# stm233/image-compression-for-machine

Measured on AMD Instinct MI355X. Metric: images/sec (256x256) cnn-hyperprior (WACNN) training step, higher is better.
Workload: dtype f32; 1 GPU; cnn (WACNN N=192 M=320) train step, lambda=0.0067 MSE, batch 16/GPU synthetic 256x256, Adam lr 1e-4 + aux Adam, clip 1.0; global_batch=16, parallelism=dp1

## Files before the change

image-compression-for-machine_amd/csrc/conv_1x1.hip:

```cpp
#include <cstdlib>
#include "conv_common.h"

namespace icm {

template <int TCO, int TPX>
__global__ __launch_bounds__(256, 2) void conv1x1_kernel(const ConvDesc d) {
  constexpr int DB = 4;
  const int lane = threadIdx.x & 63;
  const int wave = __builtin_amdgcn_readfirstlane((int)(threadIdx.x >> 6));
  const ConvPtrs P = d.g[blockIdx.y];
  int bid = xcd_block_id();
  const int cb = bid % d.ncb, ptile = bid / d.ncb;
  const int h = lane >> 5, l31 = lane & 31;
  const int HW = d.pg.H * d.pg.W;
  const int NP = d.pg.N * HW;
  const int p_base = (ptile * 4 + wave) * (32 * TPX);
  if (p_base >= NP) return;
  unsigned voff[TPX];
  int pn[TPX], phw[TPX];
  bool pv[TPX];
#pragma unroll
  for (int tp = 0; tp < TPX; ++tp) {
    const int p = p_base + tp * 32 + l31;
    pv[tp] = p < NP;
    const int pc = min(p, NP - 1);
    pn[tp] = pc / HW;
    phw[tp] = pc - pn[tp] * HW;
    voff[tp] = (unsigned)(pn[tp] * (int)d.pg.bs + phw[tp] + h * HW) * 4u;
  }
  f32x16 acc[TCO][TPX];
#pragma unroll
  for (int a = 0; a < TCO; ++a)
#pragma unroll
    for (int b = 0; b < TPX; ++b)
#pragma unroll
      for (int r = 0; r < 16; ++r) acc[a][b][r] = 0.0f;

  const char* xb = reinterpret_cast<const char*>(P.x);
  const char* wbase = reinterpret_cast<const char*>(P.wp);
  const long long cstride = (long long)HW * 4;
  const int cot0 = cb * TCO;
  unsigned wl[TCO];
#pragma unroll
  for (int a = 0; a < TCO; ++a) wl[a] = (unsigned)(min(cot0 + a, d.ncot - 1) * 64 + lane) * 16u;
  const long long qstride = (long long)d.ncot * 64 * 16;
  const int nq = d.nchunks8;
  const int act = d.pg.act;

  float bq[DB][4][TPX];
  f32x4 aq[2][TCO];
  auto loadB = [&](float (&dst)[4][TPX], int q) {
    const char* sb = xb + (long long)min(q, nq - 1) * 8 * cstride;
#pragma unroll
    for (int j = 0; j < 4; ++j)
#pragma unroll
      for (int tp = 0; tp < TPX; ++tp) dst[j][tp] = *reinterpret_cast<const float*>(sb + 2 * j * cstride + voff[tp]);
  };
#pragma unroll
  for (int a = 0; a < TCO; ++a) {
    aq[0][a] = *reinterpret_cast<const f32x4*>(wbase + wl[a]);
    aq[1][a] = *reinterpret_cast<const f32x4*>(wbase + (long long)min(1, nq - 1) * qstride + wl[a]);
  }
#pragma unroll
  for (int u = 0; u < DB; ++u) loadB(bq[u], u);

  for (int q0 = 0; q0 < nq; q0 += DB) {
#pragma unroll
    for (int u = 0; u < DB; ++u) {
      const int q = q0 + u;
      if (q >= nq) break;
      float bv[4][TPX];
#pragma unroll
      for (int j = 0; j < 4; ++j)
#pragma unroll
        for (int tp = 0; tp < TPX; ++tp) bv[j][tp] = bq[u][j][tp];
      if (act == ICM_ACT_GELU) {
#pragma unroll
        for (int j = 0; j < 4; ++j)
#pragma unroll
          for (int tp = 0; tp < TPX; ++tp) bv[j][tp] = gelu_f(bv[j][tp]);
      } else if (act == ICM_ACT_SQUARE) {
#pragma unroll
        for (int j = 0; j < 4; ++j)
#pragma unroll
          for (int tp = 0; tp < TPX; ++tp) bv[j][tp] *= bv[j][tp];
      }
      loadB(bq[u], q + DB);
      const char* sp = wbase + (long long)min(q + 2, nq - 1) * qstride;
#pragma unroll
      for (int a = 0; a < TCO; ++a) {
#pragma unroll
        for (int tp = 0; tp < TPX; ++tp)
#pragma unroll
          for (int j = 0; j < 4; ++j)
            acc[a][tp] = __builtin_amdgcn_mfma_f32_32x32x2f32(aq[u & 1][a][j], bv[j][tp], acc[a][tp], 0, 0, 0);
        aq[u & 1][a] = *reinterpret_cast<const f32x4*>(sp + wl[a]);
        __builtin_amdgcn_sched_barrier(0);
      }
    }
  }

  int zero[TPX];
#pragma unroll
  for (int tp = 0; tp < TPX; ++tp) zero[tp] = 0;
  epilogue_dispatch<TCO, TPX, !(TCO == 3 && TPX == 2)>(d, P, acc, cot0, h, pn, zero, phw, pv);
}

struct Cfg1x1 {
  int tco, tpx;
  void (*fn)(const ConvDesc);
  float eff;
};
static const Cfg1x1 kCfgs1x1[] = {
    {6, 1, conv1x1_kernel<6, 1>, 1.0f},  {5, 1, conv1x1_kernel<5, 1>, 1.0f}, {4, 1, conv1x1_kernel<4, 1>, 0.97f},
    {3, 2, conv1x1_kernel<3, 2>, 1.0f},  {2, 2, conv1x1_kernel<2, 2>, 0.7f}, {1, 2, conv1x1_kernel<1, 2>, 0.6f},
    {3, 1, conv1x1_kernel<3, 1>, 0.95f}, {2, 1, conv1x1_kernel<2, 1>, 0.6f},
};

int plan_conv1x1(const icm_conv_args& a, int ngroups, int g_force_1x1, ConvPlan& p) {
  if (g_force_1x1 == 0) return -1;
  if (a.KH != 1 || a.KW != 1 || a.stride != 1 || a.pad != 0 || a.pixel_shuffle || (a.Cin % 8) != 0) return -1;
  if (a.OH != a.H || a.OW != a.W) return -1;
  const int ncot = cdiv(a.Cout, 32);
  const long long NP = (long long)a.N * a.H * a.W;
  int best = -1, best_pad = 1 << 30;
  const int ncfg = (int)(sizeof(kCfgs1x1) / sizeof(kCfgs1x1[0]));
  for (int i = 0; i < ncfg; ++i) best_pad = std::min(best_pad, cdiv(ncot, kCfgs1x1[i].tco) * kCfgs1x1[i].tco);
  float best_score = -1.0f;
  for (int i = 0; i < ncfg; ++i) {
    const Cfg1x1& k = kCfgs1x1[i];
    if (cdiv(ncot, k.tco) * k.tco != best_pad) continue;
    const long long waves = ((NP + 32 * k.tpx - 1) / (32 * k.tpx)) * cdiv(ncot, k.tco) * ngroups;
    const float score = (float)std::min<long long>(waves, 2048) * k.eff;
    if (score > best_score) {
      best_score = score;
      best = i;
    }
  }
  {
    static const int force = env_int("ICM_1X1_CFG", -1);
    if (force >= 0 && force < ncfg) best = force;
  }
  const Cfg1x1& c = kCfgs1x1[best];
  const int ncb = cdiv(ncot, c.tco);
  const long long strips = (NP + 32 * c.tpx - 1) / (32 * c.tpx);
  static const long long kMinWaves = env_ll("ICM_1X1_MIN_WAVES", 1024);
  static const int kShortK = env_int("ICM_1X1_SHORT_K", 384);
  const long long need = a.Cin <= kShortK ? kMinWaves / 2 : kMinWaves;
  if (g_force_1x1 < 0 && strips * ncb * ngroups < need) return -1;
  const long long nblk = ((strips + 3) / 4) * ncb;
  if (nblk <= 0 || nblk > 0x7fffffffLL) return ICM_ERR_ARG;
  p = ConvPlan{};
  p.family = kFam1x1; p.row = best; p.g.ckm = 1; p.ncb = ncb; p.nblk = nblk; p.block = 256;
  return ICM_OK;
}

int launch_conv1x1(ConvDesc& d, const icm_conv_args& a, const ConvPlan& p, int ngroups, hipStream_t stream) {
  d.pg.H = a.H; d.pg.W = a.W; d.pg.N = a.N; d.pg.C = a.Cin; d.pg.act = a.pro_act; d.pg.bs = a.x_bs;
  d.OHf = a.H; d.OWf = a.W; d.OHv = a.H; d.OWv = a.W;
  d.out_sy = d.out_sx = 1;
  d.ntaps = 1;
  d.tiles_x = d.tiles_y = d.tiles_n = 1;
  d.nchunks8 = a.Cin / 8; d.ckm = p.g.ckm;
  hipLaunchKernelGGL(kCfgs1x1[p.row].fn, dim3((unsigned)p.nblk, ngroups, 1), dim3(p.block), 0, stream, d);
  ICM_CHECK_LAUNCH();
  return ICM_OK;
}

}
```

image-compression-for-machine_amd/csrc/conv_common.h:

```cpp
#pragma once
#include <type_traits>
#include "icm_common.h"

namespace icm {

#define ICM_MAX_TAPS 32
#define ICM_MAX_GROUPS 12

struct ConvPtrs {
  const float* x;
  const float* wp;
  const float* bias;
  float* y;
  const float* res;
  const float* aux;
  const float* aux2;
  float* y2;
};

struct ConvDesc {
  ConvPtrs g[ICM_MAX_GROUPS];
  long long y_bs, res_bs, aux_bs, aux2_bs, y2_bs;
  PatchGeom pg;
  int Cout, OHf, OWf;
  int OHv, OWv;
  int out_sy, out_oy, out_sx, out_ox;
  int iy0, ix0;
  int ntaps;
  int lgTW, lgTH, lgTI;
  int tiles_x, tiles_y, tiles_n;
  int ncot, nchunks8, ckm, ncb;
  int epi, accum, ps2;
  int tapoff[ICM_MAX_TAPS];
};

inline void fill_conv_ptrs(ConvPtrs (&g)[ICM_MAX_GROUPS], const icm_conv_args* arr, int ngroups, long long wp_off) {
  for (int gi = 0; gi < ICM_MAX_GROUPS; ++gi) {
    const icm_conv_args& s = arr[gi < ngroups ? gi : 0];
    g[gi] = ConvPtrs{s.x, s.wp + wp_off, s.bias, s.y, s.res, s.aux, s.aux2, s.y2};
  }
}
inline void fill_conv_desc(ConvDesc& d, const icm_conv_args* arr, int ngroups, long long wp_off) {
  const icm_conv_args& a = arr[0];
  fill_conv_ptrs(d.g, arr, ngroups, wp_off);
  d.y_bs = a.y_bs; d.res_bs = a.res_bs; d.aux_bs = a.aux_bs; d.aux2_bs = a.aux2_bs; d.y2_bs = a.y2_bs;
  d.Cout = a.Cout; d.ncot = (a.Cout + 31) / 32;
  d.epi = a.epi; d.accum = a.accum;
}

enum ConvFamily { kFamStaged = 0, kFamKs8 = 1, kFam1x1 = 2, kFamWino44 = 3, kFamWino8 = 4 };
struct Geometry {
  int lgTW, lgTH, lgTI, PH, PW, PWh, PWrow, PP, CS, tiles_x, tiles_y, tiles_n, ckm;
  size_t lds_bytes;
};
struct ConvPlan {
  int family;
  int row;
  Geometry g;
  int ncb;
  long long nblk;
  int block, vec4, dma;
};
struct WinoGeom {
  int lgTX, lgTY, lgTI, tiles_x, tiles_y, tiles_n, nchunks8, nsteps;
};
struct WinoPlan {
  WinoGeom g;
  int tco, w8, px_fast, ncb;
  long long nblk;
  size_t lds_bytes;
};

constexpr bool epi_reads_res(int e) { return e == ICM_EPI_RES || e == ICM_EPI_RES_GELU || e == ICM_EPI_RES_MUL_DGELU; }
constexpr bool epi_reads_aux(int e) {
  return e == ICM_EPI_GDN || e == ICM_EPI_IGDN || e == ICM_EPI_MUL_DGELU || e == ICM_EPI_AXPY2 || e == ICM_EPI_LRP ||
         e == ICM_EPI_RES_MUL_DGELU;
}
constexpr bool epi_reads_aux2(int e) { return e == ICM_EPI_AXPY2; }
constexpr bool epi_writes_side(int e) { return e == ICM_EPI_GDN || e == ICM_EPI_IGDN || e == ICM_EPI_LRP; }
constexpr bool epi_may_gelu(int e) { return e == ICM_EPI_NONE || e == ICM_EPI_RES || e == ICM_EPI_RES_GELU; }

template <int EPI>
__device__ __forceinline__ float epi_apply(float v, float rv, float av, float& side) {
  if constexpr (EPI == ICM_EPI_RES) v += rv;
  if constexpr (EPI == ICM_EPI_RES_GELU) v += gelu_f(rv);
  if constexpr (EPI == ICM_EPI_GDN || EPI == ICM_EPI_IGDN) {
    side = v;
    v = av * (EPI == ICM_EPI_GDN ? rsqrtf(v) : sqrtf(v));
  }
  if constexpr (EPI == ICM_EPI_MUL_DGELU) v *= dgelu_f(av);
  if constexpr (EPI == ICM_EPI_RES_MUL_DGELU) v = (v + rv) * dgelu_f(av);
  if constexpr (EPI == ICM_EPI_AXPY2) v = rv + 2.0f * av * v;
  if constexpr (EPI == ICM_EPI_LRP) {
    side = tanhf(v);
    v = av + 0.5f * side;
  }
  return v;
}
template <class Off>
__device__ __forceinline__ void epi_materialise(float& v, const float* y, float* y2, Off off, bool ok) {
  const float gv = gelu_f(v);
  if (y2 == y) v = gv;
  else if (ok) y2[off] = gv;
}

template <int... Kinds>
struct EpiKinds {
  static constexpr bool has(int epi) { return ((epi == Kinds) || ...); }
  template <class F>
  static __device__ __forceinline__ void dispatch(int epi, F&& f) {
    static_assert(((Kinds == ICM_EPI_NONE) || ...), "ICM_EPI_NONE is the fallback of every kernel");
    const bool hit = ((Kinds != ICM_EPI_NONE && epi == Kinds ? (f(std::integral_constant<int, Kinds>{}), true) : false) || ...);
    if (!hit) f(std::integral_constant<int, ICM_EPI_NONE>{});
  }
};
using EpiAll = EpiKinds<ICM_EPI_NONE, ICM_EPI_RES, ICM_EPI_RES_GELU, ICM_EPI_GDN, ICM_EPI_IGDN, ICM_EPI_MUL_DGELU,
                        ICM_EPI_AXPY2, ICM_EPI_LRP, ICM_EPI_RES_MUL_DGELU>;
using EpiKs8 = EpiKinds<ICM_EPI_NONE, ICM_EPI_RES, ICM_EPI_RES_GELU, ICM_EPI_MUL_DGELU, ICM_EPI_LRP, ICM_EPI_RES_MUL_DGELU>;
using EpiWino = EpiKinds<ICM_EPI_NONE, ICM_EPI_RES, ICM_EPI_RES_GELU, ICM_EPI_MUL_DGELU, ICM_EPI_RES_MUL_DGELU, ICM_EPI_LRP>;

template <int EPI, int half>
__device__ __forceinline__ void store_half_e(const ConvDesc& d, const ConvPtrs& P, const f32x16 acc, int cot, int h,
                                             int n, int oy, int ox, bool pvalid) {
  const int plane = d.OHf * d.OWf;
  constexpr bool kRes = epi_reads_res(EPI), kAux = epi_reads_aux(EPI), kAux2 = epi_reads_aux2(EPI);
  float* yb = P.y + n * d.y_bs;
  const float* resb = kRes ? P.res + n * d.res_bs : nullptr;
  const float* auxb = kAux ? P.aux + n * d.aux_bs : nullptr;
  const float* aux2b = kAux2 ? P.aux2 + n * d.aux2_bs : nullptr;
  float* y2b = P.y2 ? P.y2 + n * d.y2_bs : nullptr;
  const bool has_bias = P.bias != nullptr;
  {
    int off[8];
    bool ok[8];
    float bv[8], rv[8], av[8];
#pragma unroll
    for (int q = 0; q < 8; ++q) {
      const int r = half * 8 + q;
      const int co = cot * 32 + (r & 3) + 8 * (r >> 2) + 4 * h;
      ok[q] = pvalid && co < d.Cout;
      off[q] = d.ps2 ? (co >> 2) * plane + (oy * 2 + ((co >> 1) & 1)) * d.OWf + ox * 2 + (co & 1)
                     : co * plane + oy * d.OWf + ox;
      bv[q] = (has_bias && ok[q]) ? P.bias[co] : 0.0f;
      if constexpr (kRes) rv[q] = ok[q] ? resb[off[q]] : 0.0f;
      if constexpr (kAux) av[q] = ok[q] ? auxb[off[q]] : 0.0f;
      if constexpr (kAux2) rv[q] = ok[q] ? aux2b[off[q]] : 0.0f;
    }
    float v[8];
#pragma unroll
    for (int q = 0; q < 8; ++q) {
      float side;
      v[q] = epi_apply<EPI>(acc[half * 8 + q] + bv[q], (kRes || kAux2) ? rv[q] : 0.0f, kAux ? av[q] : 0.0f, side);
      if constexpr (epi_writes_side(EPI))
        if (y2b && ok[q]) y2b[off[q]] = side;
    }
    if (d.accum) {
      float old[8];
#pragma unroll
      for (int q = 0; q < 8; ++q) old[q] = ok[q] ? yb[off[q]] : 0.0f;
#pragma unroll
      for (int q = 0; q < 8; ++q) v[q] += old[q];
    }
    if constexpr (epi_may_gelu(EPI)) {
      if (y2b) {
#pragma unroll
        for (int q = 0; q < 8; ++q) epi_materialise(v[q], yb, y2b, off[q], ok[q]);
      }
    }
#pragma unroll
    for (int q = 0; q < 8; ++q)
      if (ok[q]) yb[off[q]] = v[q];
  }
}
template <int EPI>
__device__ __forceinline__ void store_tile_e(const ConvDesc& d, const ConvPtrs& P, const f32x16 acc, int cot, int h,
                                             int n, int oy, int ox, bool pvalid) {
  store_half_e<EPI, 0>(d, P, acc, cot, h, n, oy, ox, pvalid);
  store_half_e<EPI, 1>(d, P, acc, cot, h, n, oy, ox, pvalid);
}

struct EpiRegs {
  int n;
  int off[8];
  bool ok[8];
  float bv[8], rv[8], av[8], old[8];
};

template <int EPI>
__device__ __forceinline__ void epi_load(const ConvDesc& d, const ConvPtrs& P, int cot, int half, int h, int n, int oy,
                                         int ox, bool pvalid, EpiRegs& R) {
  const int plane = d.OHf * d.OWf;
  constexpr bool kRes = epi_reads_res(EPI), kAux = epi_reads_aux(EPI), kAux2 = epi_reads_aux2(EPI);
  const float* yb = P.y + n * d.y_bs;
  const float* resb = kRes ? P.res + n * d.res_bs : nullptr;
  const float* auxb = kAux ? P.aux + n * d.aux_bs : nullptr;
  const float* aux2b = kAux2 ? P.aux2 + n * d.aux2_bs : nullptr;
  const bool has_bias = P.bias != nullptr;
  const bool tile_ok = pvalid && cot < d.ncot;
  R.n = n;
#pragma unroll
  for (int q = 0; q < 8; ++q) {
    const int r = half * 8 + q;
    const int co = cot * 32 + (r & 3) + 8 * (r >> 2) + 4 * h;
    R.ok[q] = tile_ok && co < d.Cout;
    R.off[q] = d.ps2 ? (co >> 2) * plane + (oy * 2 + ((co >> 1) & 1)) * d.OWf + ox * 2 + (co & 1)
                     : co * plane + oy * d.OWf + ox;
    R.bv[q] = (has_bias && R.ok[q]) ? P.bias[co] : 0.0f;
    if constexpr (kRes) R.rv[q] = R.ok[q] ? resb[R.off[q]] : 0.0f;
    if constexpr (kAux) R.av[q] = R.ok[q] ? auxb[R.off[q]] : 0.0f;
    if constexpr (kAux2) R.rv[q] = R.ok[q] ? aux2b[R.off[q]] : 0.0f;
  }
  if (d.accum) {
#pragma unroll
    for (int q = 0; q < 8; ++q) R.old[q] = R.ok[q] ? yb[R.off[q]] : 0.0f;
  }
}

template <int EPI>
__device__ __forceinline__ void epi_finish(const ConvDesc& d, const ConvPtrs& P, const float (&a8)[8], const EpiRegs& R) {
  float* yb = P.y + R.n * d.y_bs;
  float* y2b = P.y2 ? P.y2 + R.n * d.y2_bs : nullptr;
  constexpr bool kRv = epi_reads_res(EPI) || epi_reads_aux2(EPI), kAux = epi_reads_aux(EPI);
  float v[8];
#pragma unroll
  for (int q = 0; q < 8; ++q) {
    float side;
    v[q] = epi_apply<EPI>(a8[q] + R.bv[q], kRv ? R.rv[q] : 0.0f, kAux ? R.av[q] : 0.0f, side);
    if constexpr (epi_writes_side(EPI))
      if (y2b && R.ok[q]) y2b[R.off[q]] = side;
  }
  if (d.accum) {
#pragma unroll
    for (int q = 0; q < 8; ++q) v[q] += R.old[q];
  }
  if constexpr (epi_may_gelu(EPI)) {
    if (y2b) {
#pragma unroll
      for (int q = 0; q < 8; ++q) epi_materialise(v[q], yb, y2b, R.off[q], R.ok[q]);
    }
  }
#pragma unroll
  for (int q = 0; q < 8; ++q)
    if (R.ok[q]) yb[R.off[q]] = v[q];
}

template <int EPI, int TCO, int TPX, bool PIPE>
__device__ __forceinline__ void epilogue_tiles(const ConvDesc& d, const ConvPtrs& P, const f32x16 (&acc)[TCO][TPX], int cot0,
                                               int h, const int (&pn)[TPX], const int (&poy)[TPX], const int (&pox)[TPX],
                                               const bool (&pv)[TPX]) {
  if constexpr (!PIPE) {
#pragma unroll
    for (int tp = 0; tp < TPX; ++tp)
#pragma unroll
      for (int a = 0; a < TCO; ++a) {
        if (cot0 + a < d.ncot) store_tile_e<EPI>(d, P, acc[a][tp], cot0 + a, h, pn[tp], poy[tp], pox[tp], pv[tp]);
        __builtin_amdgcn_sched_barrier(0);
      }
    return;
  }
  constexpr int S = TPX * TCO * 2;
  EpiRegs R[2];
  epi_load<EPI>(d, P, cot0, 0, h, pn[0], poy[0], pox[0], pv[0], R[0]);
#pragma unroll
  for (int i = 0; i < S; ++i) {
    const int half = i & 1, a = (i >> 1) % TCO, tp = (i >> 1) / TCO;
    if (i + 1 < S) {
      const int i2 = i + 1;
      const int half2 = i2 & 1, a2 = (i2 >> 1) % TCO, tp2 = (i2 >> 1) / TCO;
      epi_load<EPI>(d, P, cot0 + a2, half2, h, pn[tp2], poy[tp2], pox[tp2], pv[tp2], R[i2 & 1]);
    }
    __builtin_amdgcn_sched_barrier(0);
    float a8[8];
#pragma unroll
    for (int q = 0; q < 8; ++q) a8[q] = acc[a][tp][half * 8 + q];
    epi_finish<EPI>(d, P, a8, R[i & 1]);
    __builtin_amdgcn_sched_barrier(0);
  }
}

template <int TCO, int TPX, bool PIPE2 = false>
__device__ __forceinline__ void epilogue_dispatch(const ConvDesc& d, const ConvPtrs& P, const f32x16 (&acc)[TCO][TPX],
                                                  int cot0, int h, const int (&pn)[TPX], const int (&poy)[TPX],
                                                  const int (&pox)[TPX], const bool (&pv)[TPX]) {
  EpiAll::dispatch(d.epi, [&](auto kind) {
    constexpr int EPI = decltype(kind)::value;
    epilogue_tiles<EPI, TCO, TPX, EPI == ICM_EPI_AXPY2 && PIPE2>(d, P, acc, cot0, h, pn, poy, pox, pv);
  });
}

int launch_conv_ks8(const ConvDesc& d, int tco, long long nblk, int ngroups, size_t lds_bytes, hipStream_t stream);

bool wino_supported(const icm_conv_args& a);
int plan_conv_wino(const icm_conv_args& a, int ngroups, WinoPlan& p);
int run_conv_wino(const icm_conv_args* arr, int ngroups, hipStream_t stream);
long long wino_transform_floats(const icm_conv_args& a);
int run_wino_transform(const icm_conv_args* arr, int ngroups, hipStream_t stream);

int plan_conv1x1(const icm_conv_args& a, int ngroups, int force_mode, ConvPlan& p);
int launch_conv1x1(ConvDesc& d, const icm_conv_args& a, const ConvPlan& p, int ngroups, hipStream_t stream);

}
```

image-compression-for-machine_amd/csrc/conv_ks8.hip:

```cpp
#include <cstdlib>
#include "conv_common.h"

namespace icm {

template <int EPI>
__device__ __forceinline__ void ks8_store(const ConvDesc& d, const ConvPtrs& P, const f32x16 v, int cot, int hf, int h, int n,
                                          int oy, int ox, bool pvalid) {
  if (hf == 0) store_half_e<EPI, 0>(d, P, v, cot, h, n, oy, ox, pvalid);
  else store_half_e<EPI, 1>(d, P, v, cot, h, n, oy, ox, pvalid);
}

template <int TCO, int TPX>
__global__ __launch_bounds__(512, 2) void conv_ks8_kernel(const ConvDesc d) {
  extern __shared__ __attribute__((aligned(16))) float smem[];
  static_assert(TCO * TPX == 4, "four output tiles per workgroup: one half tile per wave in the epilogue");
  const int tid = threadIdx.x, lane = tid & 63;
  const int wave = __builtin_amdgcn_readfirstlane(tid >> 6);
  const ConvPtrs P = d.g[blockIdx.y];
  const PatchGeom& pg = d.pg;
  int bid = xcd_block_id();
  const int cb = bid % d.ncb;
  int pt = bid / d.ncb;
  const int tx_i = pt % d.tiles_x;
  pt /= d.tiles_x;
  const int ty_i = pt % d.tiles_y;
  const int tn_i = pt / d.tiles_y;
  const int ox0 = tx_i << d.lgTW, oy0 = ty_i << d.lgTH, n0 = tn_i << d.lgTI;
  const int iyb = oy0 + d.iy0, ixb = ox0 + d.ix0;
  const int bufsz = d.ckm * 8 * pg.CS;
  const int nchunks = (d.nchunks8 + d.ckm - 1) / d.ckm;
  const long long HWb = (long long)pg.H * pg.W * 4;
  const float* zero = icm_zero_page + lane;
  const int nj = (pg.TIPH * pg.PW + 63) >> 6;

  PlaneMap pm;
  plane_map_init(pm, pg, n0, iyb, ixb, lane);
  const char* xb = reinterpret_cast<const char*>(P.x);
  auto stage = [&](int chunk) {
    const int c0 = chunk * d.ckm * 8;
    const int nch = min(d.ckm, d.nchunks8 - chunk * d.ckm) * 8;
    float* dst = smem + (chunk & 1) * bufsz;
    for (int cl = wave; cl < nch; cl += 8) {
      const int c = c0 + cl;
      const char* base = xb + (long long)c * HWb;
      float* slab = dst + cl * pg.CS;
#pragma unroll
      for (int j = 0; j < ICM_MAXJ; ++j) {
        if (j < nj && pm.loff[j] >= 0) {
          const float* pp = (c < pg.C && pm.goff[j] >= 0) ? reinterpret_cast<const float*>(base + pm.goff[j]) : zero;
          __builtin_amdgcn_global_load_lds(pp, slab + 64 * j, 4, 0, 0);
        }
      }
    }
  };

  const int h = lane >> 5, l31 = lane & 31;
  const int TWm = (1 << d.lgTW) - 1, THm = (1 << d.lgTH) - 1;
  int boff[TPX];
#pragma unroll
  for (int tp = 0; tp < TPX; ++tp) {
    const int p = tp * 32 + l31;
    const int tx = p & TWm, ty = (p >> d.lgTW) & THm, ti = p >> (d.lgTW + d.lgTH);
    boff[tp] = h * pg.CS + ti * pg.PP + ty * pg.PWrow + tx;
  }
  f32x16 acc[TCO][TPX];
#pragma unroll
  for (int a = 0; a < TCO; ++a)
#pragma unroll
    for (int b = 0; b < TPX; ++b)
#pragma unroll
      for (int r = 0; r < 16; ++r) acc[a][b][r] = 0.0f;

  const char* wbase = reinterpret_cast<const char*>(P.wp);
  const int cot0 = cb * TCO;
  unsigned wl[TCO];
#pragma unroll
  for (int a = 0; a < TCO; ++a) wl[a] = (unsigned)(min(cot0 + a, d.ncot - 1) * 64 + lane) * 16u;
  const long long qstride = (long long)d.ncot * 64 * 16;
  const int Qtot = d.nchunks8 * d.ntaps;
  const int qchunk = d.ckm * d.ntaps;
  int step_lane;
  {
    const int sq = lane / d.ntaps, tq = lane - sq * d.ntaps;
    step_lane = sq * 8 * pg.CS + d.tapoff[tq];
  }
  constexpr int PF = 4;
  f32x4 aq[PF][TCO];
#pragma unroll
  for (int u = 0; u < PF; ++u)
#pragma unroll
    for (int a = 0; a < TCO; ++a)
      aq[u][a] = *reinterpret_cast<const f32x4*>(wbase + (long long)min(wave + 8 * u, Qtot - 1) * qstride + wl[a]);

  stage(0);
  asm volatile("s_waitcnt vmcnt(0)" ::: "memory");
  __syncthreads();
  int chunk = 0, qend = min(qchunk, Qtot);
  if (nchunks > 1) stage(1);
  auto cross = [&]() {
    asm volatile("s_waitcnt vmcnt(0)" ::: "memory");
    __syncthreads();
    ++chunk;
    qend = min((chunk + 1) * qchunk, Qtot);
    if (chunk + 1 < nchunks) stage(chunk + 1);
  };
  for (int q0 = wave; q0 < Qtot; q0 += 8 * PF) {
#pragma unroll
    for (int u = 0; u < PF; ++u) {
      const int q = q0 + 8 * u;
      if (q >= Qtot) break;
      while (q >= qend) cross();
      const float* bp = smem + (chunk & 1) * bufsz + __builtin_amdgcn_readlane(step_lane, q - chunk * qchunk);
      float bv[4][TPX];
#pragma unroll
      for (int j = 0; j < 4; ++j)
#pragma unroll
        for (int tp = 0; tp < TPX; ++tp) bv[j][tp] = bp[boff[tp] + 2 * j * pg.CS];
      const char* sp = wbase + (long long)min(q + 8 * PF, Qtot - 1) * qstride;
#pragma unroll
      for (int a = 0; a < TCO; ++a) {
#pragma unroll
        for (int tp = 0; tp < TPX; ++tp)
#pragma unroll
          for (int j = 0; j < 4; ++j)
            acc[a][tp] = __builtin_amdgcn_mfma_f32_32x32x2f32(aq[u][a][j], bv[j][tp], acc[a][tp], 0, 0, 0);
        aq[u][a] = *reinterpret_cast<const f32x4*>(sp + wl[a]);
      }
    }
  }
  while (chunk + 1 < nchunks) cross();
  asm volatile("s_waitcnt vmcnt(0)" ::: "memory");
  __syncthreads();

  float* red = smem;
#pragma unroll
  for (int a = 0; a < TCO; ++a)
#pragma unroll
    for (int tp = 0; tp < TPX; ++tp)
#pragma unroll
      for (int r = 0; r < 16; ++r) red[((wave * 4 + a * TPX + tp) * 16 + r) * 64 + lane] = acc[a][tp][r];
  __syncthreads();
  const int t = wave >> 1, hf = wave & 1;
  f32x16 v;
#pragma unroll
  for (int r = 0; r < 16; ++r) v[r] = 0.0f;
#pragma unroll
  for (int q = 0; q < 8; ++q) {
    float s = 0.0f;
#pragma unroll
    for (int k = 0; k < 8; ++k) s += red[((k * 4 + t) * 16 + hf * 8 + q) * 64 + lane];
    if (hf == 0) v[q] = s; else v[8 + q] = s;
  }
  const int a_t = t / TPX, tp_t = t % TPX;
  const int cot = cot0 + a_t;
  const int p = tp_t * 32 + l31;
  const int tx = p & TWm, ty = (p >> d.lgTW) & THm, ti = p >> (d.lgTW + d.lgTH);
  const int n = n0 + ti, oyv = oy0 + ty, oxv = ox0 + tx;
  const bool pvalid = (n < pg.N) && (oyv < d.OHv) && (oxv < d.OWv) && cot < d.ncot;
  const int oy = oyv * d.out_sy + d.out_oy, ox = oxv * d.out_sx + d.out_ox;
  EpiKs8::dispatch(d.epi, [&](auto kind) { ks8_store<decltype(kind)::value>(d, P, v, cot, hf, h, n, oy, ox, pvalid); });
}

int launch_conv_ks8(const ConvDesc& d, int tco, long long nblk, int ngroups, size_t lds_bytes, hipStream_t stream) {
  void (*fn)(const ConvDesc) = tco == 2 ? conv_ks8_kernel<2, 2> : conv_ks8_kernel<1, 4>;
  if (lds_bytes > 64 * 1024 && !ensure_max_lds(reinterpret_cast<const void*>(fn))) return ICM_ERR_LAUNCH;
  hipLaunchKernelGGL(fn, dim3((unsigned)nblk, ngroups, 1), dim3(512), lds_bytes, stream, d);
  ICM_CHECK_LAUNCH();
  return ICM_OK;
}

}
```

Measured before the change: 392.2 images/s.

## Use inline-asm loads with explicit vmcnt waits to pipeline 1x1 and ks8 conv

Replaces compiler-generated global loads in the 1x1 and split-K convolution kernels with inline-asm global_load instructions and hand-counted s_waitcnt vmcnt values. The aim is for MFMA work to wait only for the specific weight or activation registers it needs, not a full vmcnt(0). The ks8 kernel also drops full drains at LDS chunk crossings in favour of partial waits that keep weight prefetches in flight. The risk is correctness: the counts depend on exact instruction ordering and could become wrong if the compiler inserts or reorders other memory operations.

```diff
diff --git a/image-compression-for-machine_amd/csrc/conv_1x1.hip b/image-compression-for-machine_amd/csrc/conv_1x1.hip
--- a/image-compression-for-machine_amd/csrc/conv_1x1.hip
+++ b/image-compression-for-machine_amd/csrc/conv_1x1.hip
@@ -4,8 +4,51 @@
 namespace icm {
 
 template <int TCO, int TPX>
+struct Pw1x1Pipe {
+  static constexpr int DB = 4;
+  static constexpr int DA = 2;
+  static constexpr int NB = 4 * TPX;
+  static constexpr int W_TILE = DA * (TCO + NB) - 1;
+  static constexpr int W_FIRST = W_TILE - NB;
+  static_assert(DB % DA == 0 && DB >= DA, "the loop is unrolled DB chunks per trip and indexes both rings statically");
+};
+
+template <int TPX>
+__device__ __forceinline__ void pw_load_b(float (&b)[4][TPX], const unsigned (&voff)[TPX], const char* base, long long step) {
+#pragma unroll
+  for (int j = 0; j < 4; ++j) {
+    const char* sb = base + j * step;
+    if constexpr (TPX == 1)
+      asm volatile("s_nop 4\n\tglobal_load_dword %0, %1, %2" : "=&v"(b[j][0]) : "v"(voff[0]), "s"(sb) : "memory");
+    else
+      asm volatile("s_nop 4\n\tglobal_load_dword %0, %2, %4\n\tglobal_load_dword %1, %3, %4"
+                   : "=&v"(b[j][0]), "=&v"(b[j][1]) : "v"(voff[0]), "v"(voff[1]), "s"(sb) : "memory");
+  }
+}
+template <int N, int TPX>
+__device__ __forceinline__ void pw_wait_first(f32x4& a0, float (&b)[4][TPX]) {
+  static_assert(N >= 0 && N <= 63, "vmcnt is a 6-bit field");
+  static_assert(TPX == 1 || TPX == 2, "");
+  if constexpr (TPX == 1)
+    asm volatile("s_waitcnt vmcnt(%5)\n\ts_nop 1"
+                 : "+v"(a0), "+v"(b[0][0]), "+v"(b[1][0]), "+v"(b[2][0]), "+v"(b[3][0]) : "n"(N) : "memory");
+  else
+    asm volatile("s_waitcnt vmcnt(%9)\n\ts_nop 1"
+                 : "+v"(a0), "+v"(b[0][0]), "+v"(b[0][1]), "+v"(b[1][0]), "+v"(b[1][1]), "+v"(b[2][0]), "+v"(b[2][1]),
+                   "+v"(b[3][0]), "+v"(b[3][1]) : "n"(N) : "memory");
+}
+template <int TPX>
+__device__ __forceinline__ void pw_hold(float (&b)[4][TPX]) {
+#pragma unroll
+  for (int j = 0; j < 4; ++j)
+#pragma unroll
+    for (int tp = 0; tp < TPX; ++tp) asm volatile("" : "+v"(b[j][tp]));
+}
+
+template <int TCO, int TPX>
 __global__ __launch_bounds__(256, 2) void conv1x1_kernel(const ConvDesc d) {
-  constexpr int DB = 4;
+  using PL = Pw1x1Pipe<TCO, TPX>;
+  constexpr int DB = PL::DB, DA = PL::DA;
   const int lane = threadIdx.x & 63;
   const int wave = __builtin_amdgcn_readfirstlane((int)(threadIdx.x >> 6));
   const ConvPtrs P = d.g[blockIdx.y];
@@ -48,57 +91,79 @@
   const int act = d.pg.act;
 
   float bq[DB][4][TPX];
-  f32x4 aq[2][TCO];
+  f32x4 aq[DA][TCO];
   auto loadB = [&](float (&dst)[4][TPX], int q) {
-    const char* sb = xb + (long long)min(q, nq - 1) * 8 * cstride;
+    pw_load_b<TPX>(dst, voff, xb + (long long)min(q, nq - 1) * 8 * cstride, 2 * cstride);
+  };
+  auto aptr = [&](int q) -> const char* { return wbase + (long long)min(q, nq - 1) * qstride; };
+#pragma unroll
+  for (int i = -DB; i < 0; ++i) {
+    loadB(bq[i + DB], i + DB);
+    if (i + DA >= 0) {
+      const char* sp = aptr(i + DA);
+#pragma unroll
+      for (int a = 0; a < TCO; ++a) ring_load16(aq[i + DA][a], wl[a], sp);
+    }
+  }
+  __builtin_amdgcn_sched_barrier(0);
+
+  auto chunk = [&](auto u_tag, int q) {
+    constexpr int u = decltype(u_tag)::value;
+    pw_wait_first<PL::W_FIRST, TPX>(aq[u % DA][0], bq[u]);
+    float bv[4][TPX];
 #pragma unroll
     for (int j = 0; j < 4; ++j)
 #pragma unroll
-      for (int tp = 0; tp < TPX; ++tp) dst[j][tp] = *reinterpret_cast<const float*>(sb + 2 * j * cstride + voff[tp]);
+      for (int tp = 0; tp < TPX; ++tp) bv[j][tp] = bq[u][j][tp];
+    if (act == ICM_ACT_GELU) {
+#pragma unroll
+      for (int j = 0; j < 4; ++j)
+#pragma unroll
+        for (int tp = 0; tp < TPX; ++tp) bv[j][tp] = gelu_f(bv[j][tp]);
+    } else if (act == ICM_ACT_SQUARE) {
+#pragma unroll
+      for (int j = 0; j < 4; ++j)
+#pragma unroll
+        for (int tp = 0; tp < TPX; ++tp) bv[j][tp] *= bv[j][tp];
+    }
+    loadB(bq[u], q + DB);
+    __builtin_amdgcn_sched_barrier(0);
+    const char* sp = aptr(q + DA);
+#pragma unroll
+    for (int a = 0; a < TCO; ++a) {
+      if (a > 0) ring_wait<PL::W_TILE>(aq[u % DA][a]);
+#pragma unroll
+      for (int tp = 0; tp < TPX; ++tp)
+#pragma unroll
+        for (int j = 0; j < 4; ++j)
+          acc[a][tp] = __builtin_amdgcn_mfma_f32_32x32x2f32(aq[u % DA][a][j], bv[j][tp], acc[a][tp], 0, 0, 0);
+      ring_load16(aq[u % DA][a], wl[a], sp);
+      __builtin_amdgcn_sched_barrier(0);
+    }
   };
-#pragma unroll
-  for (int a = 0; a < TCO; ++a) {
-    aq[0][a] = *reinterpret_cast<const f32x4*>(wbase + wl[a]);
-    aq[1][a] = *reinterpret_cast<const f32x4*>(wbase + (long long)min(1, nq - 1) * qstride + wl[a]);
-  }
-#pragma unroll
-  for (int u = 0; u < DB; ++u) loadB(bq[u], u);
-
-  for (int q0 = 0; q0 < nq; q0 += DB) {
-#pragma unroll
-    for (int u = 0; u < DB; ++u) {
-      const int q = q0 + u;
-      if (q >= nq) break;
-      float bv[4][TPX];
-#pragma unroll
-      for (int j = 0; j < 4; ++j)
-#pragma unroll
-        for (int tp = 0; tp < TPX; ++tp) bv[j][tp] = bq[u][j][tp];
-      if (act == ICM_ACT_GELU) {
-#pragma unroll
-        for (int j = 0; j < 4; ++j)
-#pragma unroll
-          for (int tp = 0; tp < TPX; ++tp) bv[j][tp] = gelu_f(bv[j][tp]);
-      } else if (act == ICM_ACT_SQUARE) {
-#pragma unroll
-        for (int j = 0; j < 4; ++j)
-#pragma unroll
-          for (int tp = 0; tp < TPX; ++tp) bv[j][tp] *= bv[j][tp];
-      }
-      loadB(bq[u], q + DB);
-      const char* sp = wbase + (long long)min(q + 2, nq - 1) * qstride;
-#pragma unroll
-      for (int a = 0; a < TCO; ++a) {
-#pragma unroll
-        for (int tp = 0; tp < TPX; ++tp)
-#pragma unroll
-          for (int j = 0; j < 4; ++j)
-            acc[a][tp] = __builtin_amdgcn_mfma_f32_32x32x2f32(aq[u & 1][a][j], bv[j][tp], acc[a][tp], 0, 0, 0);
-        aq[u & 1][a] = *reinterpret_cast<const f32x4*>(sp + wl[a]);
-        __builtin_amdgcn_sched_barrier(0);
-      }
-    }
-  }
+  int q0 = 0;
+  for (; q0 + DB <= nq; q0 += DB) {
+    chunk(std::integral_constant<int, 0>{}, q0);
+    chunk(std::integral_constant<int, 1>{}, q0 + 1);
+    chunk(std::integral_constant<int, 2>{}, q0 + 2);
+    chunk(std::integral_constant<int, 3>{}, q0 + 3);
+  }
+  static_assert(DB == 4, "the trips above and the tail below are written out for four chunks");
+  if (q0 < nq) {
+    chunk(std::integral_constant<int, 0>{}, q0);
+    if (q0 + 1 < nq) {
+      chunk(std::integral_constant<int, 1>{}, q0 + 1);
+      if (q0 + 2 < nq) chunk(std::integral_constant<int, 2>{}, q0 + 2);
+    }
+  }
+  asm volatile("s_waitcnt vmcnt(0)" ::: "memory");
+#pragma unroll
+  for (int u = 0; u < DB; ++u) pw_hold<TPX>(bq[u]);
+#pragma unroll
+  for (int u = 0; u < DA; ++u)
+#pragma unroll
+    for (int a = 0; a < TCO; ++a) asm volatile("" : "+v"(aq[u][a]));
+  __builtin_amdgcn_sched_barrier(0);
 
   int zero[TPX];
 #pragma unroll
diff --git a/image-compression-for-machine_amd/csrc/conv_common.h b/image-compression-for-machine_amd/csrc/conv_common.h
--- a/image-compression-for-machine_amd/csrc/conv_common.h
+++ b/image-compression-for-machine_amd/csrc/conv_common.h
@@ -288,6 +288,15 @@
   });
 }
 
+__device__ __forceinline__ void ring_load16(f32x4& q, unsigned voff, const char* base) {
+  asm volatile("s_nop 4\n\tglobal_load_dwordx4 %0, %1, %2" : "=&v"(q) : "v"(voff), "s"(base) : "memory");
+}
+template <int N>
+__device__ __forceinline__ void ring_wait(f32x4& q) {
+  static_assert(N >= 0 && N <= 63, "vmcnt is a 6-bit field");
+  asm volatile("s_waitcnt vmcnt(%1)\n\ts_nop 1" : "+v"(q) : "n"(N) : "memory");
+}
+
 int launch_conv_ks8(const ConvDesc& d, int tco, long long nblk, int ngroups, size_t lds_bytes, hipStream_t stream);
 
 bool wino_supported(const icm_conv_args& a);
diff --git a/image-compression-for-machine_amd/csrc/conv_ks8.hip b/image-compression-for-machine_amd/csrc/conv_ks8.hip
--- a/image-compression-for-machine_amd/csrc/conv_ks8.hip
+++ b/image-compression-for-machine_amd/csrc/conv_ks8.hip
@@ -8,6 +8,13 @@
                                           int oy, int ox, bool pvalid) {
   if (hf == 0) store_half_e<EPI, 0>(d, P, v, cot, h, n, oy, ox, pvalid);
   else store_half_e<EPI, 1>(d, P, v, cot, h, n, oy, ox, pvalid);
+}
+
+template <int N>
+__device__ __forceinline__ void ks8_barrier() {
+  static_assert(N <= 63, "vmcnt is a 6-bit field");
+  if constexpr (N < 0) asm volatile("s_waitcnt lgkmcnt(0)\n\ts_barrier" ::: "memory");
+  else asm volatile("s_waitcnt vmcnt(%0) lgkmcnt(0)\n\ts_barrier" ::"n"(N) : "memory");
 }
 
 template <int TCO, int TPX>
@@ -85,24 +92,35 @@
     step_lane = sq * 8 * pg.CS + d.tapoff[tq];
   }
   constexpr int PF = 4;
+  constexpr int W_TILE = PF * TCO - 1;
   f32x4 aq[PF][TCO];
-#pragma unroll
-  for (int u = 0; u < PF; ++u)
-#pragma unroll
-    for (int a = 0; a < TCO; ++a)
-      aq[u][a] = *reinterpret_cast<const f32x4*>(wbase + (long long)min(wave + 8 * u, Qtot - 1) * qstride + wl[a]);
-
   stage(0);
-  asm volatile("s_waitcnt vmcnt(0)" ::: "memory");
-  __syncthreads();
+#pragma unroll
+  for (int u = 0; u < PF; ++u) {
+    const char* sp = wbase + (long long)min(wave + 8 * u, Qtot - 1) * qstride;
+#pragma unroll
+    for (int a = 0; a < TCO; ++a) ring_load16(aq[u][a], wl[a], sp);
+  }
+  ks8_barrier<PF * TCO>();
   int chunk = 0, qend = min(qchunk, Qtot);
+  int since = 0;
   if (nchunks > 1) stage(1);
-  auto cross = [&]() {
-    asm volatile("s_waitcnt vmcnt(0)" ::: "memory");
-    __syncthreads();
+  auto advance = [&]() {
     ++chunk;
     qend = min((chunk + 1) * qchunk, Qtot);
+    since = 0;
     if (chunk + 1 < nchunks) stage(chunk + 1);
+  };
+  auto cross = [&]() {
+    static_assert(PF == 4, "one case per n < PF");
+    switch (since) {
+      case 0: ks8_barrier<0>(); break;
+      case 1: ks8_barrier<TCO>(); break;
+      case 2: ks8_barrier<2 * TCO>(); break;
+      case 3: ks8_barrier<3 * TCO>(); break;
+      default: ks8_barrier<-1>(); break;
+    }
+    advance();
   };
   for (int q0 = wave; q0 < Qtot; q0 += 8 * PF) {
 #pragma unroll
@@ -119,17 +137,27 @@
       const char* sp = wbase + (long long)min(q + 8 * PF, Qtot - 1) * qstride;
 #pragma unroll
       for (int a = 0; a < TCO; ++a) {
+        ring_wait<W_TILE>(aq[u][a]);
 #pragma unroll
         for (int tp = 0; tp < TPX; ++tp)
 #pragma unroll
           for (int j = 0; j < 4; ++j)
             acc[a][tp] = __builtin_amdgcn_mfma_f32_32x32x2f32(aq[u][a][j], bv[j][tp], acc[a][tp], 0, 0, 0);
-        aq[u][a] = *reinterpret_cast<const f32x4*>(sp + wl[a]);
+        ring_load16(aq[u][a], wl[a], sp);
+        __builtin_amdgcn_sched_barrier(0);
       }
+      ++since;
     }
   }
-  while (chunk + 1 < nchunks) cross();
+  while (chunk + 1 < nchunks) {
+    ks8_barrier<0>();
+    advance();
+  }
   asm volatile("s_waitcnt vmcnt(0)" ::: "memory");
+#pragma unroll
+  for (int u = 0; u < PF; ++u)
+#pragma unroll
+    for (int a = 0; a < TCO; ++a) asm volatile("" : "+v"(aq[u][a]));
   __syncthreads();
 
   float* red = smem;
```

Result: no change. 391.3 images/s (-0.2%).
